# nsdumont/Semantic-Spiking-Neural-SLAM-2023

Measured on AMD Instinct MI355X. Metric: sim-sec/wall-sec, SSP-SLAM ssp_dim=1015 10k PI neurons, 1/2/4/8 MI355X, higher is better.
Workload: dtype f32; 1 GPU; PathIntegration 2-D ssp_dim=1015 pi_n_neurons=10000/VCO (508 VCOs, 5080000 LIF neurons), configs[1]; eval_points_per_vco=4000, parallelism=1 GPU, build_cache=miss

## Files before the change

semantic-spiking-neural-slam-2023_amd/csrc/ssn_block.hpp:

```cpp
#pragma once
#include <type_traits>
#include "ssn_launch.hpp"

namespace ssn {

__device__ inline float wave_sum_dpp(float v) {
  int x;
#define SSN_DPP_ADD(ctrl, rmask)                                                                             \
  x = __builtin_amdgcn_update_dpp(0, __builtin_bit_cast(int, v), ctrl, rmask, 0xF, false);                    \
  v += __builtin_bit_cast(float, x);
  SSN_DPP_ADD(0xB1, 0xF)
  SSN_DPP_ADD(0x4E, 0xF)
  SSN_DPP_ADD(0x141, 0xF)
  SSN_DPP_ADD(0x140, 0xF)
  SSN_DPP_ADD(0x142, 0xA)
  SSN_DPP_ADD(0x143, 0xC)
#undef SSN_DPP_ADD
  return v;
}
__device__ inline float row_sum_dpp(float v) {
  int x;
#define SSN_DPP_ADD(ctrl)                                                                                    \
  x = __builtin_amdgcn_update_dpp(0, __builtin_bit_cast(int, v), ctrl, 0xF, 0xF, false);                      \
  v += __builtin_bit_cast(float, x);
  SSN_DPP_ADD(0xB1) SSN_DPP_ADD(0x4E) SSN_DPP_ADD(0x141) SSN_DPP_ADD(0x140)
#undef SSN_DPP_ADD
  return v;
}
template <int N>
__device__ inline void wave_sum_dpp_n(float* v) {
#define SSN_DPP_STAGE(ctrl, rmask)                                                                            \
  _Pragma("unroll") for (int r = 0; r < N; ++r) {                                                              \
    const int x = __builtin_amdgcn_update_dpp(0, __builtin_bit_cast(int, v[r]), ctrl, rmask, 0xF, false);      \
    v[r] += __builtin_bit_cast(float, x);                                                                      \
  }
  SSN_DPP_STAGE(0xB1, 0xF) SSN_DPP_STAGE(0x4E, 0xF) SSN_DPP_STAGE(0x141, 0xF) SSN_DPP_STAGE(0x140, 0xF)
  SSN_DPP_STAGE(0x142, 0xA) SSN_DPP_STAGE(0x143, 0xC)
#undef SSN_DPP_STAGE
}
__device__ inline double wave_sum_dpp(double v) {
#pragma unroll
  for (int off = 32; off > 0; off >>= 1) v += __shfl_xor(v, off, 64);
  return v;
}
template <int N>
__device__ inline void wave_sum_dpp_n(double* v) {
#pragma unroll
  for (int r = 0; r < N; ++r) v[r] = wave_sum_dpp(v[r]);
}

typedef float f32x2 __attribute__((ext_vector_type(2)));
typedef unsigned int u32x2 __attribute__((ext_vector_type(2)));
__device__ inline f32x2 pk_clamp01(f32x2 x) {
  f32x2 r;
  asm("v_pk_mul_f32 %0, %1, 1.0 op_sel_hi:[1,0] clamp" : "=v"(r) : "v"(x));
  return r;
}
__device__ inline f32x2 pk_sub_clamp01(f32x2 x, f32x2 y) {
  f32x2 r;
  asm("v_pk_add_f32 %0, %1, %2 neg_lo:[0,1] neg_hi:[0,1] clamp" : "=v"(r) : "v"(x), "s"(y));
  return r;
}
__device__ inline f32x2 pk_mul_clamp01(f32x2 x, f32x2 y) {
  f32x2 r;
  asm("v_pk_mul_f32 %0, %1, %2 clamp" : "=v"(r) : "v"(x), "s"(y));
  return r;
}
__device__ inline f32x2 pk_fma_clamp01_vsv(f32x2 x, f32x2 y, f32x2 z) {
  f32x2 r;
  asm("v_pk_fma_f32 %0, %1, %2, %3 clamp" : "=v"(r) : "v"(x), "s"(y), "v"(z));
  return r;
}
__device__ inline f32x2 pk_fma_clamp01_trans_vvs(f32x2 x, f32x2 y, f32x2 z) {
  f32x2 r;
  asm("s_nop 0\n\tv_pk_fma_f32 %0, %1, %2, %3 clamp" : "=v"(r) : "v"(x), "v"(y), "s"(z));
  return r;
}

__device__ inline f32x2 pk_fma_clamp01_vs_negv(f32x2 x, f32x2 y, f32x2 z) {
  f32x2 r;
  asm("v_pk_fma_f32 %0, %1, %2, %3 neg_lo:[0,0,1] neg_hi:[0,0,1] clamp" : "=v"(r) : "v"(x), "s"(y), "v"(z));
  return r;
}

struct LifConstV3 { float na, ca, m1, c1, c2, c3, p0, p1, p2, ktau_ref, K; };

__device__ inline LifConstV3 lif_const_v3(double dt, double tau_rc, double tau_ref) {
  double K = 1.0;
  while (2.0 * K * tau_ref <= 1.0 && K < 1048576.0) K *= 2.0;
  while (K * tau_ref > 1.0) K *= 0.5;
  const double h = dt / tau_rc;
  const double x0 = h, x1 = 0.5 * h, x2 = 0.0669872981077807 * h;
  auto f = [](double x) { return -expm1(-x) / x; };
  const double f0 = f(x0), f1 = f(x1), f2 = f(x2);
  const double d01 = (f1 - f0) / (x1 - x0), d12 = (f2 - f1) / (x2 - x1), d012 = (d12 - d01) / (x2 - x0);
  const double q2 = d012, q1 = d01 - d012 * (x0 + x1), q0 = f0 - d01 * x0 + d012 * x0 * x1;
  LifConstV3 c;
  const float a = (float)(1.0 / (K * dt));
  float ca = a + 1.0f;
  if ((double)ca < (double)a + 1.0) ca = __builtin_bit_cast(float, __builtin_bit_cast(unsigned int, ca) + 1u);
  c.na = -a; c.ca = ca; c.m1 = (float)(1.0 + K * dt);
  c.c1 = (float)(q0 * h); c.c2 = (float)(q1 * h * h); c.c3 = (float)(q2 * h * h * h);
  {
    const double um = -expm1(-h);
    const double u0 = um * 0.9330127018922193, u1 = um * 0.5, u2 = um * 0.0669872981077807;
    auto phi = [](double u) { return log1p(-u) / u; };
    const double g0 = phi(u0), g1 = phi(u1), g2 = phi(u2);
    const double e01 = (g1 - g0) / (u1 - u0), e12 = (g2 - g1) / (u2 - u1), e012 = (e12 - e01) / (u2 - u0);
    const double r2 = e012, r1 = e01 - e012 * (u0 + u1), r0 = g0 - e01 * u0 + e012 * u0 * u1;
    c.p0 = (float)(K * tau_rc * r0); c.p1 = (float)(K * tau_rc * r1); c.p2 = (float)(K * tau_rc * r2);
  }
  c.ktau_ref = (float)(K * tau_ref); c.K = (float)K;
  return c;
}

__device__ inline void lif_state_part(f32x2 w, const LifConstV3& c, f32x2& W0, f32x2& em) {
  W0 = pk_clamp01(w);
  const f32x2 dl = pk_fma_clamp01_vsv(w, (f32x2)(c.na), (f32x2)(c.ca));
  f32x2 P;
  asm("v_pk_fma_f32 %0, %1, %2, %3" : "=v"(P) : "v"(dl), "v"((f32x2)(c.c3)), "s"((f32x2)(c.c2)));
  asm("v_pk_fma_f32 %0, %1, %2, %3" : "=v"(P) : "v"(dl), "v"(P), "s"((f32x2)(c.c1)));
  em = dl * P;
}
__device__ inline f32x2 lif_spike_test(f32x2 Jm1, f32x2 w, f32x2 W0, f32x2 em, const LifConstV3& c, f32x2 big, f32x2& U, f32x2& nmt) {
  nmt = pk_sub_clamp01(w, (f32x2)(c.m1));
  U = __builtin_elementwise_fma(Jm1 + W0, em, -W0);
  return pk_mul_clamp01(U, big);
}
__device__ inline void lif_finish_spiking(f32x2 Jm1, f32x2& w, f32x2 U, f32x2 nmt, f32x2 spk, const LifConstV3& c, f32x2 big) {
  f32x2 rc;
  rc.x = __builtin_amdgcn_rcpf(Jm1.x);
  rc.y = __builtin_amdgcn_rcpf(Jm1.y);
  const f32x2 u = U * rc;
  f32x2 P, nu;
  asm("v_pk_fma_f32 %0, %1, %2, %3" : "=v"(P) : "v"(u), "v"((f32x2)(c.p2)), "s"((f32x2)(c.p1)));
  asm("v_pk_fma_f32 %0, %1, %2, %3" : "=v"(P) : "v"(u), "v"(P), "s"((f32x2)(c.p0)));
  asm("v_pk_fma_f32 %0, %1, %2, %3 clamp" : "=v"(nu) : "v"(u), "v"(P), "s"((f32x2)(c.ktau_ref)));
  const f32x2 Wn = pk_fma_clamp01_vs_negv(spk, big, U);
  w = __builtin_elementwise_fma(spk, nu, Wn + nmt);
}
__device__ inline void lif_finish_silent(f32x2& w, f32x2 U, f32x2 nmt) {
  f32x2 Wn;
  asm("v_pk_mul_f32 %0, %1, -1.0 op_sel_hi:[1,0] clamp" : "=v"(Wn) : "v"(U));
  w = Wn + nmt;
}
__device__ inline f32x2 lif_input_part(f32x2 Jm1, f32x2& w, f32x2 W0, f32x2 em, const LifConstV3& c, f32x2 big) {
  const f32x2 nmt = pk_sub_clamp01(w, (f32x2)(c.m1));
  const f32x2 U = __builtin_elementwise_fma(Jm1 + W0, em, -W0);
  const f32x2 spk = pk_mul_clamp01(U, big);
  f32x2 rc;
  rc.x = __builtin_amdgcn_rcpf(Jm1.x);
  rc.y = __builtin_amdgcn_rcpf(Jm1.y);
  f32x2 Wn, u, P, nu;
  asm("v_pk_fma_f32 %0, %2, %3, %4 neg_lo:[0,0,1] neg_hi:[0,0,1] clamp\n\t"
      "v_pk_mul_f32 %1, %4, %5"
      : "=&v"(Wn), "=v"(u)
      : "v"(spk), "s"(big), "v"(U), "v"(rc));
  asm("v_pk_fma_f32 %0, %1, %2, %3" : "=v"(P) : "v"(u), "v"((f32x2)(c.p2)), "s"((f32x2)(c.p1)));
  asm("v_pk_fma_f32 %0, %1, %2, %3" : "=v"(P) : "v"(u), "v"(P), "s"((f32x2)(c.p0)));
  asm("v_pk_fma_f32 %0, %1, %2, %3 clamp" : "=v"(nu) : "v"(u), "v"(P), "s"((f32x2)(c.ktau_ref)));
  w = __builtin_elementwise_fma(spk, nu, Wn + nmt);
  return spk;
}
__device__ inline float lif_word_in(float s, float K) { return __builtin_fmaf(-s, s < 0.0f ? K : 1.0f, 1.0f); }
__device__ inline float lif_word_out(float w, float K) { return (1.0f - w) * (w > 1.0f ? 1.0f / K : 1.0f); }

__device__ inline float bits_f(unsigned int x) { return __builtin_bit_cast(float, x); }
__device__ inline unsigned int f_bits(float x) { return __builtin_bit_cast(unsigned int, x); }

#ifdef SSN_BLOCK_STAMPS
__device__ unsigned long long g_block_stamps[8];
inline hipError_t read_block_stamps(unsigned long long* out, int reset) {
  hipError_t e = hipMemcpyFromSymbol(out, HIP_SYMBOL(g_block_stamps), sizeof(unsigned long long) * 8);
  if (e == hipSuccess && reset) {
    const unsigned long long z[8] = {0, 0, 0, 0, 0, 0, 0, 0};
    e = hipMemcpyToSymbol(HIP_SYMBOL(g_block_stamps), z, sizeof z);
  }
  return e;
}
#define SSN_BSTAMP(var)                                                                          \
  do {                                                                                           \
    __builtin_amdgcn_sched_barrier(0);                                                           \
    asm volatile("s_memtime %0\n\ts_waitcnt lgkmcnt(0)" : "=s"(var) :: "memory");                \
    __builtin_amdgcn_sched_barrier(0);                                                           \
  } while (0)
#define SSN_BSTAMP_ADD(i, a, b) bst[i] += (b) - (a)
#else
#define SSN_BSTAMP(var) do {} while (0)
#define SSN_BSTAMP_ADD(i, a, b) do {} while (0)
#endif

template <typename T, int DIN, int DOUT, int NPT, int TPB, int LDSW, int SPLIT = 0>
__global__ __launch_bounds__(TPB) void k_ens_block(BlockArgs<T> a) {
  constexpr bool ENC_LDS = LDSW == DIN;
  static_assert(LDSW == 0 || LDSW == DIN, "LDSW");
  extern __shared__ __align__(16) unsigned char ssn_block_dyn[];
  T* const e_lds = reinterpret_cast<T*>(ssn_block_dyn);
  constexpr bool F32 = sizeof(T) == 4;
  constexpr int PK = F32 ? 2 : 1;
  constexpr int NG = NPT / PK;
  static_assert(NPT % PK == 0, "f32 variants handle neuron pairs");
  using G = typename std::conditional<F32, f32x2, T>::type;
  constexpr int DP = DOUT <= 4 ? 4 : 8;
  static_assert(!SPLIT || (sizeof(T) == 4 && DOUT <= 4), "split ensembles: f32, at most four decoded rows");
  const int P = SPLIT ? a.P : 1;
  const int k = P > 1 ? (int)blockIdx.x / P : (int)blockIdx.x;
  const int member = P > 1 ? (int)blockIdx.x - k * P : 0;
  const int noff = member * a.n_member;
  const int n_loc = P > 1 ? max(0, min(a.n_member, a.n_pad - noff)) : a.n_pad;
  const int tid = threadIdx.x;
  const int nthr = NG == 1 ? (int)blockDim.x : TPB;
  const int lane = tid & 63, wave = tid >> 6;
  const size_t row = (size_t)a.n_pad;
  const T* __restrict__ enc = a.enc + (size_t)k * DIN * row + noff;
  const T* __restrict__ bias = a.bias + (size_t)k * row + noff;
  T* __restrict__ Sp = a.S + (size_t)k * row + noff;
  const NeuronParams<T> np = a.np;
  const LifMath<T> lm(np);
  auto uni = [](float v) { return bits_f(__builtin_amdgcn_readfirstlane(f_bits(v))); };
  LifConstV3 lc = lif_const_v3((double)np.dt, (double)np.tau_rc, (double)np.tau_ref);
  lc.na = uni(lc.na); lc.ca = uni(lc.ca); lc.m1 = uni(lc.m1); lc.c1 = uni(lc.c1); lc.c2 = uni(lc.c2); lc.c3 = uni(lc.c3); lc.p0 = uni(lc.p0); lc.p1 = uni(lc.p1); lc.p2 = uni(lc.p2); lc.ktau_ref = uni(lc.ktau_ref);
  lc.K = uni(lc.K);
  const f32x2 big = {0x1p100f, 0x1p100f};

  G e[ENC_LDS ? 1 : NG][DIN], b[NG], s[NG], dc[NG][DOUT];
  constexpr int cap = (NG == 1 ? 1024 : TPB) * NPT;
  int lrow[LDSW > 0 ? LDSW : 1];
#pragma unroll
  for (int d = 0; d < (LDSW > 0 ? LDSW : 1); ++d) {
    lrow[d] = d * cap + tid * PK;
    asm volatile("" : "+v"(lrow[d]));
  }
  auto lds_group = [&](int d, int g) -> const G* {
    return reinterpret_cast<const G*>(e_lds + lrow[d] + g * nthr * PK);
  };
#pragma unroll
  for (int g = 0; g < NG; ++g) {
    const int i0 = (g * nthr + tid) * PK;
    const bool in = i0 < n_loc;
    const int ii = in ? i0 : 0;
    const T msk = in ? T(1) : T(0);
    auto ld = [&](const T* p) -> G { if constexpr (F32) return *reinterpret_cast<const f32x2*>(p) * msk; else return *p * msk; };
#pragma unroll
    for (int d = 0; d < DIN; ++d) {
      const G ev = ld(enc + d * row + ii);
      if constexpr (ENC_LDS) *reinterpret_cast<G*>(e_lds + d * cap + i0) = ev; else e[g][d] = ev;
    }
    b[g] = ld(bias + ii);
    s[g] = ld(Sp + ii);
    if constexpr (F32) {
      b[g] = b[g] - 1.0f;
      s[g] = (f32x2){lif_word_in(s[g].x, lc.K), lif_word_in(s[g].y, lc.K)};
    }
    if (a.dec_neuron_major) {
      const T* dp = a.dec + ((size_t)k * row + noff + ii) * DP;
#pragma unroll
      for (int r = 0; r < DOUT; ++r) {
        if constexpr (F32) dc[g][r] = (f32x2){dp[r], dp[DP + r]} * msk; else dc[g][r] = dp[r] * msk;
      }
    } else {
      const T* dp = a.dec + (size_t)k * DOUT * row + noff + ii;
#pragma unroll
      for (int r = 0; r < DOUT; ++r) dc[g][r] = ld(dp + r * row);
    }
  }

  constexpr int CH = 32;
  constexpr int XP = 4;
  constexpr int RW = DOUT <= 4 ? 64 : 128;
  __shared__ __align__(16) T red[2][RW];
  __shared__ __align__(16) T xs[CH][XP];
  __shared__ T os[CH][DOUT];
  __shared__ int s_dst[DOUT];
  __shared__ int s_out[DOUT];
  for (int i = tid; i < 2 * RW; i += nthr) (&red[0][0])[i] = T(0);
  if (tid < DOUT) { s_dst[tid] = a.didx[(long long)k * DOUT + tid]; s_out[tid] = a.rowout[(long long)k * DOUT + tid] ? 1 : 0; }
  const T* __restrict__ xbase = a.xrows + (size_t)a.row0 * a.n_sig + a.x_off + (long long)k * DIN;

  T fs[F32 ? 1 : DOUT], la[F32 ? 1 : DOUT], lb[F32 ? 1 : DOUT], tot[F32 ? 1 : DOUT];
  float F0 = 0.0f, F1 = 0.0f, la0 = 0.0f, lb0 = 0.0f, la1 = 0.0f, lb1 = 0.0f, v0 = 0.0f, v1 = 0.0f;
  T xa[DIN];
  int xr[DIN];
#pragma unroll
  for (int d = 0; d < DIN; ++d) {
    xr[d] = a.xrow[(long long)k * DIN + d];
    xa[d] = xr[d] >= 0 ? a.xalpha[(long long)k * DIN + d] : T(0);
  }
  if constexpr (F32) {
    const int r0 = lane >> 4;
    if (r0 < DOUT) {
      const long long i = (long long)k * DOUT + r0;
      const int st = a.lp_state[i];
      if (st >= 0) { F0 = a.sig[st]; la0 = a.lp_a[i]; lb0 = a.lp_b[i]; }
    }
    if (DOUT > 4) {
      const long long i = (long long)k * DOUT + 4;
      const int st = a.lp_state[i];
      if (st >= 0) { F1 = a.sig[st]; la1 = a.lp_a[i]; lb1 = a.lp_b[i]; }
    }
  } else {
#pragma unroll
    for (int r = 0; r < DOUT; ++r) {
      const long long i = (long long)k * DOUT + r;
      const int st = a.lp_state[i];
      fs[r] = st >= 0 ? a.sig[st] : T(0);
      la[r] = st >= 0 ? a.lp_a[i] : T(0);
      lb[r] = st >= 0 ? a.lp_b[i] : T(0);
      tot[r] = T(0);
    }
  }
  int wslot = -1;
  if constexpr (F32) {
    if constexpr (DOUT >= 4) {
      const int rv = (lane >> 4) == 1 ? 2 : ((lane >> 4) == 2 ? 1 : (lane >> 4));
      if ((lane & 15) == 0) wslot = rv * 16 + wave;
      if (DOUT == 5 && lane == 63) wslot = 64 + wave;
    }
  }

  constexpr int ILE = F32 ? (SSN_BLOCK_IL < NG ? SSN_BLOCK_IL : NG) : 1;
  G en[ILE][LDSW > 0 ? LDSW : 1];
  if constexpr (ENC_LDS) {
#pragma unroll
    for (int u = 0; u < ILE; ++u)
#pragma unroll
      for (int d = 0; d < LDSW; ++d) en[u][d] = *lds_group(d, u);
  }
#ifdef SSN_BLOCK_STAMPS
  unsigned long long bst[5] = {0, 0, 0, 0, 0}, bt0 = 0, bt1 = 0, bt2 = 0, bt3 = 0, bt4 = 0, bt5 = 0, bm0 = 0, br0 = 0;
  asm volatile("s_memtime %0\n\ts_memrealtime %1\n\ts_waitcnt lgkmcnt(0)" : "=s"(bm0), "=s"(br0) :: "memory");
#endif
  unsigned int n_slots = 0, n_silent = 0;
  for (int j0 = 0; j0 < a.B; j0 += CH) {
    const int cn = min(CH, a.B - j0);
    __syncthreads();
    if (j0 > 0 && member == 0) {
      for (int i = tid; i < CH * DOUT; i += nthr) {
        const int jj = i / DOUT, r = i - jj * DOUT;
        if (s_out[r]) a.bsig[(size_t)(a.row0 + j0 - CH + jj) * a.n_sig + s_dst[r]] = os[jj][r];
      }
    }
    for (int i = tid; i < cn * DIN; i += nthr) {
      const int jj = i / DIN, d = i - jj * DIN;
      xs[jj][d] = xbase[(size_t)(j0 + jj) * a.n_sig + d];
    }
    __syncthreads();

    for (int jj = 0; jj < cn; ++jj) {
      SSN_BSTAMP(bt0);
      if constexpr (SPLIT != 0) {
        if (P > 1 && wave == 0 && (lane & 15) == 0) {
          unsigned int* const rst = a.xslots + (size_t)k * 64 + (size_t)((j0 + jj + 1) % 3) * ((size_t)a.K * 64) + member * 4 + (lane >> 4);
          const unsigned int sent = BLOCK_XCHG_SENTINEL;
          asm volatile("global_store_dword %0, %1, off sc0 sc1" :: "v"(rst), "v"(sent) : "memory");
        }
      }
      T xin[XP];
      if constexpr (sizeof(T) == 4) *(float4*)xin = *(const float4*)xs[jj];
      else { *(double2*)xin = *(const double2*)xs[jj]; *(double2*)(xin + 2) = *(const double2*)(xs[jj] + 2); }
      T x[DIN];
      if constexpr (F32) {
        float f1 = 0.0f;
        if constexpr (DOUT > 4) f1 = bits_f(__builtin_amdgcn_readlane(f_bits(F1), 0));
#pragma unroll
        for (int d = 0; d < DIN; ++d) {
          const float f0 = bits_f(__builtin_amdgcn_readlane(f_bits(F0), (xr[d] & 3) << 4));
          float st = f0;
          if constexpr (DOUT > 4) st = xr[d] >= 4 ? f1 : f0;
          x[d] = __builtin_fmaf(xa[d], st, xin[d]);
        }
      } else {
#pragma unroll
        for (int d = 0; d < DIN; ++d) {
          T st = T(0);
#pragma unroll
          for (int r = 0; r < DOUT; ++r) st = xr[d] == r ? fs[r] : st;
          x[d] = xr[d] >= 0 ? xin[d] + xa[d] * st : xin[d];
        }
      }
      SSN_BSTAMP(bt1);
      G accg[DOUT];
#pragma unroll
      for (int r = 0; r < DOUT; ++r) accg[r] = G(0);
      constexpr int IL = ILE;
#pragma unroll
      for (int g0 = 0; g0 < NG; g0 += IL) {
        G J[IL], spk[IL];
#pragma unroll
        for (int u = 0; u < IL; ++u) {
          const int g = g0 + u < NG ? g0 + u : NG - 1;
          J[u] = b[g];
#pragma unroll
          for (int d = 0; d < DIN; ++d) {
            if constexpr (ENC_LDS) J[u] += en[u][d] * x[d];
            else J[u] += e[g][d] * x[d];
          }
        }
        if constexpr (ENC_LDS) {
#pragma unroll
          for (int u = 0; u < IL; ++u) {
            if (g0 + u >= NG) continue;
            asm volatile("" : "+v"(J[u]));
            const int gn = g0 + IL + u < NG ? g0 + IL + u : (g0 + IL + u) % IL;
#pragma unroll
            for (int d = 0; d < LDSW; ++d) en[u][d] = *lds_group(d, gn);
          }
        }
#ifndef SSN_BLOCK_SKIP
#define SSN_BLOCK_SKIP 0
#endif
        bool at_rest = false;
        if constexpr (F32 && SSN_BLOCK_SKIP == 2) {
          ++n_slots;
          f32x2 r2 = {0.0f, 0.0f};
#pragma unroll
          for (int u = 0; u < IL; ++u) {
            if (g0 + u >= NG) continue;
            f32x2 pj;
            asm("v_pk_add_f32 %0, %1, 1.0 op_sel_hi:[1,0] clamp" : "=v"(pj) : "v"(J[u]));
            const f32x2 q = s[g0 + u] - 1.0f;
            r2 += __builtin_elementwise_fma(q, q, pj);
          }
          at_rest = __builtin_amdgcn_ballot_w64(__builtin_bit_cast(unsigned long long, r2) != 0ull) == 0ull;
          if (at_rest) ++n_silent;
        }
        if constexpr (F32 && SSN_BLOCK_SKIP == 1) {
          ++n_slots;
          f32x2 Uu[IL], nm[IL];
          f32x2 any2 = {0.0f, 0.0f};
#pragma unroll
          for (int u = 0; u < IL; ++u) {
            const int g = g0 + u < NG ? g0 + u : NG - 1;
            f32x2 W0, em;
            lif_state_part(s[g], lc, W0, em);
            spk[u] = lif_spike_test(J[u], s[g], W0, em, lc, big, Uu[u], nm[u]);
            if (g0 + u < NG) any2 += spk[u];
          }
          if (__builtin_amdgcn_ballot_w64(any2.x + any2.y != 0.0f) != 0ull) {
#pragma unroll
            for (int u = 0; u < IL; ++u)
              if (g0 + u < NG) lif_finish_spiking(J[u], s[g0 + u], Uu[u], nm[u], spk[u], lc, big);
#pragma unroll
            for (int u = 0; u < IL; ++u) {
              if (g0 + u >= NG) continue;
#pragma unroll
              for (int r = 0; r < DOUT; ++r) accg[r] = __builtin_elementwise_fma(spk[u], dc[g0 + u][r], accg[r]);
            }
          } else {
#pragma unroll
            for (int u = 0; u < IL; ++u)
              if (g0 + u < NG) lif_finish_silent(s[g0 + u], Uu[u], nm[u]);
            ++n_silent;
          }
        }
        if (!at_rest) {
#pragma unroll
        for (int u = 0; u < IL; ++u) {
          const int g = g0 + u;
          if (g >= NG) continue;
          if constexpr (F32 && SSN_BLOCK_SKIP == 1) {
          } else if constexpr (F32) {
            f32x2 W0, em;
            lif_state_part(s[g], lc, W0, em);
            spk[u] = lif_input_part(J[u], s[g], W0, em, lc, big);
          } else {
            const T sw = s[g];
            T V = sw < T(0) ? T(0) : sw;
            T R = (sw < T(0) ? -sw : T(0)) - np.dt;
            T delta = np.dt - R;
            delta = delta < T(0) ? T(0) : (delta > np.dt ? np.dt : delta);
            V = V - (J[u] - V) * lm.decay(delta);
            spk[u] = T(0);
            if (V > T(1)) {
              const T t_spike = np.dt + np.tau_rc * lm.spike_time_term(V, J[u]);
              R = np.tau_ref + t_spike;
              V = T(0);
              spk[u] = T(1);
            } else if (V < T(0)) {
              V = T(0);
            }
            s[g] = R > np.dt ? -R : V;
          }
        }
#pragma unroll
        for (int u = 0; u < IL; ++u) {
          const int g = g0 + u;
          if (g >= NG) continue;
          if constexpr (F32) asm volatile("" : "+v"(s[g]));
          if constexpr (F32 && SSN_BLOCK_SKIP == 1) continue;
#pragma unroll
          for (int r = 0; r < DOUT; ++r) {
            if constexpr (F32) accg[r] = __builtin_elementwise_fma(spk[u], dc[g][r], accg[r]);
            else accg[r] = fma(spk[u], dc[g][r], accg[r]);
          }
        }
        }
#ifndef SSN_BLOCK_NO_SCHED_BARRIER
        if constexpr (F32) __builtin_amdgcn_sched_barrier(0);
#endif
      }
      const int par = jj & 1;
      SSN_BSTAMP(bt2);
      if constexpr (F32) {
        float acc[DOUT];
#pragma unroll
        for (int r = 0; r < DOUT; ++r) acc[r] = accg[r].x + accg[r].y;
        if constexpr (DOUT >= 4) {
          const auto p01 = __builtin_amdgcn_permlane32_swap(f_bits(acc[0]), f_bits(acc[1]), false, false);
          const auto p23 = __builtin_amdgcn_permlane32_swap(f_bits(acc[2]), f_bits(acc[3]), false, false);
          const float s01 = bits_f(p01[0]) + bits_f(p01[1]);
          const float s23 = bits_f(p23[0]) + bits_f(p23[1]);
          const auto q = __builtin_amdgcn_permlane16_swap(f_bits(s01), f_bits(s23), false, false);
          float t4 = bits_f(q[0]) + bits_f(q[1]);
          t4 = row_sum_dpp(t4);
          if constexpr (DOUT == 5) {
            const float w4 = wave_sum_dpp(acc[4]);
            if (wslot >= 0) red[par][wslot] = lane == 63 ? w4 : t4;
          } else {
            if (wslot >= 0) red[par][wslot] = t4;
          }
        } else {
          wave_sum_dpp_n<DOUT>(acc);
          if (lane == 63) {
#pragma unroll
            for (int r = 0; r < DOUT; ++r) red[par][r * 16 + wave] = acc[r];
          }
        }
        SSN_BSTAMP(bt3);
        __syncthreads();
        SSN_BSTAMP(bt4);
        v0 = row_sum_dpp(red[par][lane]);
        if constexpr (SPLIT != 0) {
          if (P > 1) {
            const int tq = j0 + jj;
            unsigned int* const xb = a.xslots + (size_t)k * 64;
            const size_t bstride = (size_t)a.K * 64;
            if (wave == 0 && (lane & 15) == 0) {
              unsigned int* const pub = xb + (size_t)(tq % 3) * bstride + member * 4 + (lane >> 4);
              const unsigned int val = f_bits(v0);
              asm volatile("s_waitcnt vmcnt(0)\n\tglobal_store_dword %0, %1, off sc0 sc1" :: "v"(pub), "v"(val) : "memory");
            }
            const unsigned int* const src = xb + (size_t)(tq % 3) * bstride + (lane & 15) * 4 + (lane >> 4);
            const bool mine = (lane & 15) < P;
            unsigned int got = 0, spins = 0;
            while (true) {
              if (mine) asm volatile("global_load_dword %0, %1, off sc0 sc1\n\ts_waitcnt vmcnt(0)" : "=v"(got) : "v"(src) : "memory");
              if (!__any(mine && got == BLOCK_XCHG_SENTINEL)) break;
              if (++spins > (1u << 20)) { if (lane == 0) *a.xerr = 1; break; }
            }
            v0 = row_sum_dpp(mine ? bits_f(got) : 0.0f);
          }
        }
        F0 = __builtin_fmaf(la0, F0, lb0 * v0);
        if constexpr (DOUT > 4) {
          v1 = row_sum_dpp(red[par][64 + lane]);
          F1 = __builtin_fmaf(la1, F1, lb1 * v1);
        }
        if (wave == 0 && member == 0) {
          if ((lane & 15) == 0 && (lane >> 4) < DOUT) os[jj][lane >> 4] = v0;
          if (DOUT > 4 && lane == 0) os[jj][4] = v1;
        }
        SSN_BSTAMP(bt5);
        SSN_BSTAMP_ADD(0, bt0, bt1); SSN_BSTAMP_ADD(1, bt1, bt2); SSN_BSTAMP_ADD(2, bt2, bt3); SSN_BSTAMP_ADD(3, bt3, bt4);
        SSN_BSTAMP_ADD(4, bt4, bt5);
      } else {
        T acc[DOUT];
#pragma unroll
        for (int r = 0; r < DOUT; ++r) acc[r] = accg[r];
        wave_sum_dpp_n<DOUT>(acc);
        if (lane == 63) {
#pragma unroll
          for (int r = 0; r < DOUT; ++r) red[par][r * 16 + wave] = acc[r];
        }
        __syncthreads();
#pragma unroll
        for (int r = 0; r < DOUT; ++r) {
          T t = T(0);
#pragma unroll
          for (int w = 0; w < 16; ++w) t += red[par][r * 16 + w];
          tot[r] = t;
        }
#pragma unroll
        for (int r = 0; r < DOUT; ++r) fs[r] = la[r] * fs[r] + lb[r] * tot[r];
        if (tid < DOUT) {
          T v = T(0);
#pragma unroll
          for (int r = 0; r < DOUT; ++r) v = tid == r ? tot[r] : v;
          os[jj][tid] = v;
        }
      }
    }
  }
#ifdef SSN_BLOCK_STAMPS
  if constexpr (F32) {
    unsigned long long bm1, br1;
    asm volatile("s_memtime %0\n\ts_memrealtime %1\n\ts_waitcnt lgkmcnt(0)" : "=s"(bm1), "=s"(br1) :: "memory");
    if (lane == 0) {
      for (int i = 0; i < 5; ++i) atomicAdd(&g_block_stamps[i], bst[i]);
      atomicAdd(&g_block_stamps[5], (unsigned long long)a.B);
      if (k == 0 && wave == 0) { atomicAdd(&g_block_stamps[6], bm1 - bm0); atomicAdd(&g_block_stamps[7], br1 - br0); }
    }
  }
#endif
  if constexpr (F32 && SSN_BLOCK_SKIP != 0) {
    if (lane == 0 && a.slot_stats) {
      atomicAdd(a.slot_stats, (unsigned long long)n_slots);
      atomicAdd(a.slot_stats + 1, (unsigned long long)n_silent);
    }
  }
  __syncthreads();
  if (member == 0) {
    const int j0 = (a.B - 1) / CH * CH, cn = a.B - j0;
    for (int i = tid; i < cn * DOUT; i += nthr) {
      const int jj = i / DOUT, r = i - jj * DOUT;
      if (s_out[r]) a.bsig[(size_t)(a.row0 + j0 + jj) * a.n_sig + s_dst[r]] = os[jj][r];
    }
  }

  int tid2 = tid;
  asm volatile("" : "+v"(tid2));
#pragma unroll
  for (int g = 0; g < NG; ++g) {
    const int i0 = (g * nthr + tid2) * PK;
    if constexpr (F32) s[g] = (f32x2){lif_word_out(s[g].x, lc.K), lif_word_out(s[g].y, lc.K)};
    if (i0 < n_loc) *reinterpret_cast<G*>(Sp + i0) = s[g];
  }
  if (a.B > 0 && member == 0) {
    if constexpr (F32) {
      if (wave == 0 && (lane & 15) == 0 && (lane >> 4) < DOUT) {
        const int r = lane >> 4;
        a.sig_w[s_dst[r]] = v0;
        const int st = a.lp_state[(long long)k * DOUT + r];
        if (st >= 0) a.sig_w[st] = F0;
      }
      if (DOUT > 4 && tid == 0) {
        a.sig_w[s_dst[4]] = v1;
        const int st = a.lp_state[(long long)k * DOUT + 4];
        if (st >= 0) a.sig_w[st] = F1;
      }
    } else if (tid < DOUT) {
      T v = T(0), f = T(0);
#pragma unroll
      for (int r = 0; r < DOUT; ++r) { v = tid == r ? tot[r] : v; f = tid == r ? fs[r] : f; }
      a.sig_w[s_dst[tid]] = v;
      const int st = a.lp_state[(long long)k * DOUT + tid];
      if (st >= 0) a.sig_w[st] = f;
    }
  }
}

constexpr int BLOCK_LDS_BYTES = 160 * 1024, BLOCK_STATIC_LDS = 2560;

template <typename T, int DIN, int DOUT, int NPT, int TPB, int LDSW, int SPLIT>
static hipError_t launch_block_variant_s(hipStream_t s, const BlockArgs<T>& a) {
  const int lds = LDSW * a.threads * NPT * (int)sizeof(T);
  static std::atomic<uint64_t> configured{0};
  if (LDSW > 0) {
    hipError_t e = set_max_dynamic_lds_once(reinterpret_cast<const void*>(&k_ens_block<T, DIN, DOUT, NPT, TPB, LDSW, SPLIT>),
                                            BLOCK_LDS_BYTES - BLOCK_STATIC_LDS, configured);
    if (e != hipSuccess) return e;
  }
  hipLaunchKernelGGL((k_ens_block<T, DIN, DOUT, NPT, TPB, LDSW, SPLIT>), dim3((unsigned)(a.K * (SPLIT ? a.P : 1))), dim3((unsigned)a.threads), lds, s, a);
  return hipGetLastError();
}
template <typename T, int DIN, int DOUT, int NPT, int TPB, int LDSW>
static hipError_t launch_block_variant(hipStream_t s, const BlockArgs<T>& a) {
  if (a.P > 1) {
    if constexpr (sizeof(T) == 4 && DOUT <= 4) return launch_block_variant_s<T, DIN, DOUT, NPT, TPB, LDSW, 1>(s, a);
    else return hipErrorInvalidValue;
  }
  return launch_block_variant_s<T, DIN, DOUT, NPT, TPB, LDSW, 0>(s, a);
}

struct BlockVariant { int tpb, npt, ldsw; };
template <typename T> struct BlockVariants;
template <> struct BlockVariants<float> {
  static constexpr int N = 7;
  static constexpr BlockVariant v[N] = {{1024, 2, 0}, {1024, 4, 0}, {512, 6, 0}, {1024, 6, 0}, {512, 10, 0}, {512, 20, 3}, {768, 14, 3}};
};
template <> struct BlockVariants<double> {
  static constexpr int N = 3;
  static constexpr BlockVariant v[N] = {{1024, 1, 0}, {1024, 2, 0}, {1024, 4, 0}};
};

template <typename T, int DIN, int DOUT>
static hipError_t launch_block_npt(hipStream_t s, const BlockArgs<T>& a) {
  const int key = (a.tpb * 100 + a.npt) * 8 + a.enc_lds;
  switch (key) {
#define SSN_CASE(TPB, N, L) case (TPB * 100 + N) * 8 + L: return launch_block_variant<T, DIN, DOUT, N, TPB, L>(s, a);
    SSN_CASE(1024, 2, 0) SSN_CASE(1024, 4, 0)
#undef SSN_CASE
#define SSN_CASE(TPB, N, L) case (TPB * 100 + N) * 8 + L: if constexpr (sizeof(T) == 8) return launch_block_variant<T, DIN, DOUT, N, TPB, L>(s, a); else return hipErrorInvalidValue;
    SSN_CASE(1024, 1, 0)
#undef SSN_CASE
#define SSN_CASE(TPB, N, L) case (TPB * 100 + N) * 8 + L: if constexpr (sizeof(T) == 4) return launch_block_variant<T, DIN, DOUT, N, TPB, L>(s, a); else return hipErrorInvalidValue;
    SSN_CASE(1024, 6, 0) SSN_CASE(512, 6, 0) SSN_CASE(512, 10, 0) SSN_CASE(512, 20, 3) SSN_CASE(768, 14, 3)
#undef SSN_CASE
    default: return hipErrorInvalidValue;
  }
}

template <typename T>
bool ens_block_supported(int din, int dout, int n, const int want[3], int* threads, int* tpb, int* npt, int* enc_lds) {
  if (!(din == 3 && dout >= 3 && dout <= 5)) return false;
  const int want_tpb = want[0], want_npt = want[1], want_lds = want[2];
  const int pk = sizeof(T) == 4 ? 2 : 1;
  for (int i = 0; i < BlockVariants<T>::N; ++i) {
    const BlockVariant v = BlockVariants<T>::v[i];
    if (want_tpb && (v.tpb != want_tpb || v.npt != want_npt || v.ldsw != want_lds)) continue;
    int th = v.tpb;
    if (v.npt == pk && n < th * pk) th = std::max(64, ((n + pk - 1) / pk + 63) / 64 * 64);
    if ((int64_t)th * v.npt < n) continue;
    if ((int64_t)v.ldsw * th * v.npt * (int64_t)sizeof(T) > BLOCK_LDS_BYTES - BLOCK_STATIC_LDS) continue;
    *threads = th; *tpb = v.tpb; *npt = v.npt; *enc_lds = v.ldsw;
    return true;
  }
  return false;
}

template <typename T>
hipError_t launch_ens_block(hipStream_t s, const BlockArgs<T>& a) {
  if (a.din == 3 && a.dout == 5) return launch_block_npt<T, 3, 5>(s, a);
  if (a.din == 3 && a.dout == 4) return launch_block_npt<T, 3, 4>(s, a);
  if (a.din == 3 && a.dout == 3) return launch_block_npt<T, 3, 3>(s, a);
  return hipErrorInvalidValue;
}

}
```

Before: 336.9 sim-sec/wall-sec.

## Overlap next-step LIF state and input assembly with block reduction barrier

Moves the state-dependent LIF precomputation (W0, em) for the first few neuron groups of the next timestep into the latency shadow of the cross-wave reduction. The work is placed around the __syncthreads and interleaved with the DPP row-sum in hand-written asm. It also prefetches and assembles the next step's input vector before the current step ends, and stores the LIF constants as pre-broadcast pairs. The aim is to hide barrier and reduction latency on the serial per-timestep critical path. In exchange it raises register pressure through the extra hoisted arrays and relies on fragile inline asm scheduling.

```diff
diff --git a/semantic-spiking-neural-slam-2023_amd/csrc/ssn_block.hpp b/semantic-spiking-neural-slam-2023_amd/csrc/ssn_block.hpp
--- a/semantic-spiking-neural-slam-2023_amd/csrc/ssn_block.hpp
+++ b/semantic-spiking-neural-slam-2023_amd/csrc/ssn_block.hpp
@@ -84,6 +84,7 @@
 }
 
 struct LifConstV3 { float na, ca, m1, c1, c2, c3, p0, p1, p2, ktau_ref, K; };
+struct LifConstV3P { f32x2 na, ca, m1, c1, c2, c3, p0, p1, p2, ktau_ref; };
 
 __device__ inline LifConstV3 lif_const_v3(double dt, double tau_rc, double tau_ref) {
   double K = 1.0;
@@ -114,20 +115,30 @@
   return c;
 }
 
-__device__ inline void lif_state_part(f32x2 w, const LifConstV3& c, f32x2& W0, f32x2& em) {
+__device__ inline f32x2 lif_state_dl(f32x2 w, f32x2 na, f32x2 ca) {
+  return pk_fma_clamp01_vsv(w, (f32x2)(na), (f32x2)(ca));
+}
+__device__ inline f32x2 lif_state_p1(f32x2 dl, f32x2 c3, f32x2 c2) {
+  f32x2 P;
+  asm("v_pk_fma_f32 %0, %1, %2, %3" : "=v"(P) : "v"(dl), "v"((f32x2)(c3)), "s"((f32x2)(c2)));
+  return P;
+}
+__device__ inline f32x2 lif_state_p2(f32x2 dl, f32x2 P, f32x2 c1) {
+  asm("v_pk_fma_f32 %0, %1, %2, %3" : "=v"(P) : "v"(dl), "v"(P), "s"((f32x2)(c1)));
+  return P;
+}
+__device__ inline void lif_state_part(f32x2 w, const LifConstV3P& c, f32x2& W0, f32x2& em) {
   W0 = pk_clamp01(w);
-  const f32x2 dl = pk_fma_clamp01_vsv(w, (f32x2)(c.na), (f32x2)(c.ca));
-  f32x2 P;
-  asm("v_pk_fma_f32 %0, %1, %2, %3" : "=v"(P) : "v"(dl), "v"((f32x2)(c.c3)), "s"((f32x2)(c.c2)));
-  asm("v_pk_fma_f32 %0, %1, %2, %3" : "=v"(P) : "v"(dl), "v"(P), "s"((f32x2)(c.c1)));
+  const f32x2 dl = lif_state_dl(w, c.na, c.ca);
+  const f32x2 P = lif_state_p2(dl, lif_state_p1(dl, c.c3, c.c2), c.c1);
   em = dl * P;
 }
-__device__ inline f32x2 lif_spike_test(f32x2 Jm1, f32x2 w, f32x2 W0, f32x2 em, const LifConstV3& c, f32x2 big, f32x2& U, f32x2& nmt) {
+__device__ inline f32x2 lif_spike_test(f32x2 Jm1, f32x2 w, f32x2 W0, f32x2 em, const LifConstV3P& c, f32x2 big, f32x2& U, f32x2& nmt) {
   nmt = pk_sub_clamp01(w, (f32x2)(c.m1));
   U = __builtin_elementwise_fma(Jm1 + W0, em, -W0);
   return pk_mul_clamp01(U, big);
 }
-__device__ inline void lif_finish_spiking(f32x2 Jm1, f32x2& w, f32x2 U, f32x2 nmt, f32x2 spk, const LifConstV3& c, f32x2 big) {
+__device__ inline void lif_finish_spiking(f32x2 Jm1, f32x2& w, f32x2 U, f32x2 nmt, f32x2 spk, const LifConstV3P& c, f32x2 big) {
   f32x2 rc;
   rc.x = __builtin_amdgcn_rcpf(Jm1.x);
   rc.y = __builtin_amdgcn_rcpf(Jm1.y);
@@ -144,7 +155,7 @@
   asm("v_pk_mul_f32 %0, %1, -1.0 op_sel_hi:[1,0] clamp" : "=v"(Wn) : "v"(U));
   w = Wn + nmt;
 }
-__device__ inline f32x2 lif_input_part(f32x2 Jm1, f32x2& w, f32x2 W0, f32x2 em, const LifConstV3& c, f32x2 big) {
+__device__ inline f32x2 lif_input_part(f32x2 Jm1, f32x2& w, f32x2 W0, f32x2 em, const LifConstV3P& c, f32x2 big) {
   const f32x2 nmt = pk_sub_clamp01(w, (f32x2)(c.m1));
   const f32x2 U = __builtin_elementwise_fma(Jm1 + W0, em, -W0);
   const f32x2 spk = pk_mul_clamp01(U, big);
@@ -169,11 +180,11 @@
 __device__ inline unsigned int f_bits(float x) { return __builtin_bit_cast(unsigned int, x); }
 
 #ifdef SSN_BLOCK_STAMPS
-__device__ unsigned long long g_block_stamps[8];
+__device__ unsigned long long g_block_stamps[9];
 inline hipError_t read_block_stamps(unsigned long long* out, int reset) {
-  hipError_t e = hipMemcpyFromSymbol(out, HIP_SYMBOL(g_block_stamps), sizeof(unsigned long long) * 8);
+  hipError_t e = hipMemcpyFromSymbol(out, HIP_SYMBOL(g_block_stamps), sizeof(unsigned long long) * 9);
   if (e == hipSuccess && reset) {
-    const unsigned long long z[8] = {0, 0, 0, 0, 0, 0, 0, 0};
+    const unsigned long long z[9] = {0, 0, 0, 0, 0, 0, 0, 0, 0};
     e = hipMemcpyToSymbol(HIP_SYMBOL(g_block_stamps), z, sizeof z);
   }
   return e;
@@ -190,6 +201,31 @@
 #define SSN_BSTAMP_ADD(i, a, b) do {} while (0)
 #endif
 
+#ifndef SSN_BLOCK_SKIP
+#define SSN_BLOCK_SKIP 0
+#endif
+#ifndef SSN_BLOCK_PIPE
+#define SSN_BLOCK_PIPE 1
+#endif
+#ifndef SSN_BLOCK_HOIST_A
+#define SSN_BLOCK_HOIST_A 2
+#endif
+#ifndef SSN_BLOCK_HOIST_B
+#define SSN_BLOCK_HOIST_B 4
+#endif
+#ifndef SSN_BLOCK_HOIST_C
+#define SSN_BLOCK_HOIST_C 2
+#endif
+struct BlockHoist { int a, b, c; };
+constexpr BlockHoist block_hoist(bool pipe, int tpb, int ng) {
+  if (!pipe || SSN_BLOCK_SKIP != 0) return {0, 0, 0};
+  const int room = tpb <= 512 && ng >= 10 ? ng : 0;
+  const int c = SSN_BLOCK_HOIST_C >= 2 && room >= 2 ? 2 : 0;
+  int b = SSN_BLOCK_HOIST_B < room - c ? SSN_BLOCK_HOIST_B : room - c;
+  int a_ = SSN_BLOCK_HOIST_A < room - c - b ? SSN_BLOCK_HOIST_A : room - c - b;
+  return {a_, b, c};
+}
+
 template <typename T, int DIN, int DOUT, int NPT, int TPB, int LDSW, int SPLIT = 0>
 __global__ __launch_bounds__(TPB) void k_ens_block(BlockArgs<T> a) {
   constexpr bool ENC_LDS = LDSW == DIN;
@@ -200,6 +236,9 @@
   constexpr int PK = F32 ? 2 : 1;
   constexpr int NG = NPT / PK;
   static_assert(NPT % PK == 0, "f32 variants handle neuron pairs");
+  constexpr bool PIPE = F32 && NG >= 5 && SSN_BLOCK_PIPE != 0;
+  constexpr BlockHoist HO = block_hoist(PIPE, TPB, NG);
+  constexpr int HC = HO.c, HA = HO.a, HB = HO.b, HT = HC + HA + HB;
   using G = typename std::conditional<F32, f32x2, T>::type;
   constexpr int DP = DOUT <= 4 ? 4 : 8;
   static_assert(!SPLIT || (sizeof(T) == 4 && DOUT <= 4), "split ensembles: f32, at most four decoded rows");
@@ -218,9 +257,11 @@
   const NeuronParams<T> np = a.np;
   const LifMath<T> lm(np);
   auto uni = [](float v) { return bits_f(__builtin_amdgcn_readfirstlane(f_bits(v))); };
-  LifConstV3 lc = lif_const_v3((double)np.dt, (double)np.tau_rc, (double)np.tau_ref);
-  lc.na = uni(lc.na); lc.ca = uni(lc.ca); lc.m1 = uni(lc.m1); lc.c1 = uni(lc.c1); lc.c2 = uni(lc.c2); lc.c3 = uni(lc.c3); lc.p0 = uni(lc.p0); lc.p1 = uni(lc.p1); lc.p2 = uni(lc.p2); lc.ktau_ref = uni(lc.ktau_ref);
-  lc.K = uni(lc.K);
+  const LifConstV3 lc0 = lif_const_v3((double)np.dt, (double)np.tau_rc, (double)np.tau_ref);
+  auto uni2 = [&](float v) { const float u = uni(v); return (f32x2){u, u}; };
+  const LifConstV3P lc = {uni2(lc0.na), uni2(lc0.ca), uni2(lc0.m1), uni2(lc0.c1), uni2(lc0.c2), uni2(lc0.c3), uni2(lc0.p0), uni2(lc0.p1),
+                          uni2(lc0.p2), uni2(lc0.ktau_ref)};
+  const float lcK = uni(lc0.K);
   const f32x2 big = {0x1p100f, 0x1p100f};
 
   G e[ENC_LDS ? 1 : NG][DIN], b[NG], s[NG], dc[NG][DOUT];
@@ -250,7 +291,7 @@
     s[g] = ld(Sp + ii);
     if constexpr (F32) {
       b[g] = b[g] - 1.0f;
-      s[g] = (f32x2){lif_word_in(s[g].x, lc.K), lif_word_in(s[g].y, lc.K)};
+      s[g] = (f32x2){lif_word_in(s[g].x, lcK), lif_word_in(s[g].y, lcK)};
     }
     if (a.dec_neuron_major) {
       const T* dp = a.dec + ((size_t)k * row + noff + ii) * DP;
@@ -327,10 +368,31 @@
       for (int d = 0; d < LDSW; ++d) en[u][d] = *lds_group(d, u);
   }
 #ifdef SSN_BLOCK_STAMPS
-  unsigned long long bst[5] = {0, 0, 0, 0, 0}, bt0 = 0, bt1 = 0, bt2 = 0, bt3 = 0, bt4 = 0, bt5 = 0, bm0 = 0, br0 = 0;
+  unsigned long long bst[6] = {0, 0, 0, 0, 0, 0}, bt0 = 0, bt1 = 0, bt2 = 0, bt3 = 0, bt4 = 0, bt5 = 0, bt6 = 0, bm0 = 0, br0 = 0;
   asm volatile("s_memtime %0\n\ts_memrealtime %1\n\ts_waitcnt lgkmcnt(0)" : "=s"(bm0), "=s"(br0) :: "memory");
 #endif
   unsigned int n_slots = 0, n_silent = 0;
+  T x[DIN];
+  int xl[DIN];
+#pragma unroll
+  for (int d = 0; d < DIN; ++d) xl[d] = __builtin_amdgcn_readfirstlane((xr[d] & 3) << 4);
+  auto assemble_x = [&](const float4 xv) {
+    const float xin[4] = {xv.x, xv.y, xv.z, xv.w};
+    float f1 = 0.0f;
+    if constexpr (DOUT > 4) f1 = bits_f(__builtin_amdgcn_readlane(f_bits(F1), 0));
+#pragma unroll
+    for (int d = 0; d < DIN; ++d) {
+      const float f0 = bits_f(__builtin_amdgcn_readlane(f_bits(F0), xl[d]));
+      float st = f0;
+      if constexpr (DOUT > 4) st = xr[d] >= 4 ? f1 : f0;
+      x[d] = __builtin_fmaf(xa[d], st, xin[d]);
+    }
+  };
+  f32x2 W0h[HT > 0 ? HT : 1], emh[HT > 0 ? HT : 1];
+  if constexpr (HT > 0) {
+#pragma unroll
+    for (int g = 0; g < HT; ++g) lif_state_part(s[g], lc, W0h[g], emh[g]);
+  }
   for (int j0 = 0; j0 < a.B; j0 += CH) {
     const int cn = min(CH, a.B - j0);
     __syncthreads();
@@ -345,6 +407,9 @@
       xs[jj][d] = xbase[(size_t)(j0 + jj) * a.n_sig + d];
     }
     __syncthreads();
+    if constexpr (PIPE) {
+      assemble_x(*(const float4*)xs[0]);
+    }
 
     for (int jj = 0; jj < cn; ++jj) {
       SSN_BSTAMP(bt0);
@@ -355,21 +420,12 @@
           asm volatile("global_store_dword %0, %1, off sc0 sc1" :: "v"(rst), "v"(sent) : "memory");
         }
       }
-      T xin[XP];
-      if constexpr (sizeof(T) == 4) *(float4*)xin = *(const float4*)xs[jj];
-      else { *(double2*)xin = *(const double2*)xs[jj]; *(double2*)(xin + 2) = *(const double2*)(xs[jj] + 2); }
-      T x[DIN];
-      if constexpr (F32) {
-        float f1 = 0.0f;
-        if constexpr (DOUT > 4) f1 = bits_f(__builtin_amdgcn_readlane(f_bits(F1), 0));
-#pragma unroll
-        for (int d = 0; d < DIN; ++d) {
-          const float f0 = bits_f(__builtin_amdgcn_readlane(f_bits(F0), (xr[d] & 3) << 4));
-          float st = f0;
-          if constexpr (DOUT > 4) st = xr[d] >= 4 ? f1 : f0;
-          x[d] = __builtin_fmaf(xa[d], st, xin[d]);
-        }
+      if constexpr (PIPE) {
+      } else if constexpr (F32) {
+        assemble_x(*(const float4*)xs[jj]);
       } else {
+        T xin[XP];
+        *(double2*)xin = *(const double2*)xs[jj]; *(double2*)(xin + 2) = *(const double2*)(xs[jj] + 2);
 #pragma unroll
         for (int d = 0; d < DIN; ++d) {
           T st = T(0);
@@ -406,9 +462,6 @@
             for (int d = 0; d < LDSW; ++d) en[u][d] = *lds_group(d, gn);
           }
         }
-#ifndef SSN_BLOCK_SKIP
-#define SSN_BLOCK_SKIP 0
-#endif
         bool at_rest = false;
         if constexpr (F32 && SSN_BLOCK_SKIP == 2) {
           ++n_slots;
@@ -461,7 +514,8 @@
           if constexpr (F32 && SSN_BLOCK_SKIP == 1) {
           } else if constexpr (F32) {
             f32x2 W0, em;
-            lif_state_part(s[g], lc, W0, em);
+            if (g < HT) { W0 = W0h[g < HT ? g : 0]; em = emh[g < HT ? g : 0]; }
+            else lif_state_part(s[g], lc, W0, em);
             spk[u] = lif_input_part(J[u], s[g], W0, em, lc, big);
           } else {
             const T sw = s[g];
@@ -502,6 +556,9 @@
       const int par = jj & 1;
       SSN_BSTAMP(bt2);
       if constexpr (F32) {
+        float4 xnx = {0.0f, 0.0f, 0.0f, 0.0f};
+        if constexpr (PIPE) xnx = *(const float4*)xs[jj + 1 < cn ? jj + 1 : jj];
+        (void)xnx;
         float acc[DOUT];
 #pragma unroll
         for (int r = 0; r < DOUT; ++r) acc[r] = accg[r].x + accg[r].y;
@@ -526,10 +583,51 @@
             for (int r = 0; r < DOUT; ++r) red[par][r * 16 + wave] = acc[r];
           }
         }
+        if constexpr (HA > 0) {
+          __builtin_amdgcn_sched_barrier(0);
+#pragma unroll
+          for (int g = HC; g < HC + HA; ++g) lif_state_part(s[g], lc, W0h[g], emh[g]);
+          __builtin_amdgcn_sched_barrier(0);
+        }
         SSN_BSTAMP(bt3);
         __syncthreads();
         SSN_BSTAMP(bt4);
-        v0 = row_sum_dpp(red[par][lane]);
+        if constexpr (PIPE) {
+          const float rv = red[par][lane];
+          float rv1 = 0.0f;
+          if constexpr (DOUT > 4) rv1 = red[par][64 + lane];
+          if constexpr (HB > 0) {
+            __builtin_amdgcn_sched_barrier(0);
+#pragma unroll
+            for (int g = HC + HA; g < HT; ++g) lif_state_part(s[g], lc, W0h[g], emh[g]);
+            __builtin_amdgcn_sched_barrier(0);
+          }
+          if constexpr (HC == 2) {
+            f32x2 dl0, dl1, P0, P1;
+            v0 = rv;
+            asm volatile(
+                "v_pk_fma_f32 %1, %7, %9, %10 clamp\n\t"
+                "v_pk_fma_f32 %2, %8, %9, %10 clamp\n\t"
+                "v_add_f32_dpp %0, %0, %0 quad_perm:[1,0,3,2] row_mask:0xf bank_mask:0xf bound_ctrl:1\n\t"
+                "v_pk_fma_f32 %3, %1, %11, %12\n\t"
+                "v_pk_fma_f32 %4, %2, %11, %12\n\t"
+                "v_add_f32_dpp %0, %0, %0 quad_perm:[2,3,0,1] row_mask:0xf bank_mask:0xf bound_ctrl:1\n\t"
+                "v_pk_fma_f32 %3, %1, %3, %13\n\t"
+                "v_pk_fma_f32 %4, %2, %4, %13\n\t"
+                "v_add_f32_dpp %0, %0, %0 row_half_mirror row_mask:0xf bank_mask:0xf bound_ctrl:1\n\t"
+                "v_pk_mul_f32 %5, %1, %3\n\t"
+                "v_pk_mul_f32 %6, %2, %4\n\t"
+                "v_add_f32_dpp %0, %0, %0 row_mirror row_mask:0xf bank_mask:0xf bound_ctrl:1"
+                : "+v"(v0), "=&v"(dl0), "=&v"(dl1), "=&v"(P0), "=&v"(P1), "=&v"(emh[0]), "=&v"(emh[1])
+                : "v"(s[0]), "v"(s[1]), "s"(lc.na), "v"(lc.ca), "v"(lc.c3), "s"(lc.c2), "s"(lc.c1));
+          } else {
+            v0 = row_sum_dpp(rv);
+          }
+          if constexpr (DOUT > 4) v1 = rv1;
+        } else {
+          v0 = row_sum_dpp(red[par][lane]);
+        }
+        SSN_BSTAMP(bt5);
         if constexpr (SPLIT != 0) {
           if (P > 1) {
             const int tq = j0 + jj;
@@ -552,17 +650,24 @@
           }
         }
         F0 = __builtin_fmaf(la0, F0, lb0 * v0);
+        if constexpr (HC > 0) {
+          __builtin_amdgcn_sched_barrier(0);
+#pragma unroll
+          for (int g = 0; g < HC; ++g) W0h[g] = pk_clamp01(s[g]);
+          __builtin_amdgcn_sched_barrier(0);
+        }
         if constexpr (DOUT > 4) {
-          v1 = row_sum_dpp(red[par][64 + lane]);
+          if constexpr (PIPE) v1 = row_sum_dpp(v1); else v1 = row_sum_dpp(red[par][64 + lane]);
           F1 = __builtin_fmaf(la1, F1, lb1 * v1);
         }
+        if constexpr (PIPE) assemble_x(xnx);
         if (wave == 0 && member == 0) {
           if ((lane & 15) == 0 && (lane >> 4) < DOUT) os[jj][lane >> 4] = v0;
           if (DOUT > 4 && lane == 0) os[jj][4] = v1;
         }
-        SSN_BSTAMP(bt5);
+        SSN_BSTAMP(bt6);
         SSN_BSTAMP_ADD(0, bt0, bt1); SSN_BSTAMP_ADD(1, bt1, bt2); SSN_BSTAMP_ADD(2, bt2, bt3); SSN_BSTAMP_ADD(3, bt3, bt4);
-        SSN_BSTAMP_ADD(4, bt4, bt5);
+        SSN_BSTAMP_ADD(4, bt4, bt6); SSN_BSTAMP_ADD(5, bt4, bt5);
       } else {
         T acc[DOUT];
 #pragma unroll
@@ -597,6 +702,7 @@
     asm volatile("s_memtime %0\n\ts_memrealtime %1\n\ts_waitcnt lgkmcnt(0)" : "=s"(bm1), "=s"(br1) :: "memory");
     if (lane == 0) {
       for (int i = 0; i < 5; ++i) atomicAdd(&g_block_stamps[i], bst[i]);
+      atomicAdd(&g_block_stamps[8], bst[5]);
       atomicAdd(&g_block_stamps[5], (unsigned long long)a.B);
       if (k == 0 && wave == 0) { atomicAdd(&g_block_stamps[6], bm1 - bm0); atomicAdd(&g_block_stamps[7], br1 - br0); }
     }
@@ -622,7 +728,7 @@
 #pragma unroll
   for (int g = 0; g < NG; ++g) {
     const int i0 = (g * nthr + tid2) * PK;
-    if constexpr (F32) s[g] = (f32x2){lif_word_out(s[g].x, lc.K), lif_word_out(s[g].y, lc.K)};
+    if constexpr (F32) s[g] = (f32x2){lif_word_out(s[g].x, lcK), lif_word_out(s[g].y, lcK)};
     if (i0 < n_loc) *reinterpret_cast<G*>(Sp + i0) = s[g];
   }
   if (a.B > 0 && member == 0) {
```

Result: faster. 362.0 sim-sec/wall-sec (median of 6 runs) (+7.4%).
